# numericalEFT/MCIntegration.jl

Hardware: AMD Instinct MI355X
Metric: Msamples/sec (whole node), 16-D Gaussian :vegas (higher is better)
Workload: dtype f64

## Files before the change

### mcintegration.jl_amd/_lib.py

```python
import ctypes as C
import os

_PKG = os.path.dirname(os.path.abspath(__file__))
_SO = os.path.join(_PKG, "lib", "libmci_hip.so")

MCI_OK = 0
ERR_NAMES = {1: "INVALID", 2: "HIP", 3: "COMPILE", 4: "NORMALIZATION", 5: "HISTOGRAM", 6: "COMM", 7: "NO_DEVICE"}
CONTINUOUS, DISCRETE, FERMIK = 0, 1, 2
VEGAS, VEGASMC, MCMC = 0, 1, 2
ABI_VERSION = 5
SOLVERS = {"vegas": VEGAS, "vegasmc": VEGASMC, "mcmc": MCMC, VEGAS: VEGAS, VEGASMC: VEGASMC, MCMC: MCMC}

c_double_p = C.POINTER(C.c_double)
c_int32_p = C.POINTER(C.c_int32)


class MCIError(RuntimeError):
    def __init__(self, code, msg):
        super().__init__("[MCI_ERR_%s] %s" % (ERR_NAMES.get(code, code), msg))
        self.code = code


class LeafDesc(C.Structure):
    _fields_ = [("kind", C.c_int32), ("pool", C.c_int32), ("lower", C.c_double), ("upper", C.c_double),
# ... 113 lines not shown
    ("mci_mcmc_burnin", C.c_int64, [C.c_int64, C.c_int64, C.c_int32, C.c_int32, C.c_int32, C.c_double]),
    ("mci_mcmc_auto_chains", C.c_int64, [C.c_int64, C.c_int64, C.c_int32, C.c_int32, C.c_int32, C.c_int64, C.c_int64, C.c_int32]),
    ("mci_get_hold_histogram", C.c_int, [_VP, C.POINTER(C.c_uint64)]),
    ("mci_mcmc_launch_valid", C.c_int, [_VP, c_int32_p, c_int32_p, C.POINTER(C.c_int64), C.POINTER(C.c_int64)]),
    ("mci_iteration_discard", C.c_int, [_VP]),
    ("mci_get_block_means", C.c_int, [_VP, C.c_int32, c_double_p, C.POINTER(C.c_int64), c_int32_p]),
    ("mci_reset_block_log", C.c_int, [_VP]),
    ("mci_lineage_sums", None, [c_double_p, C.c_int64, C.c_int64, C.c_int64, c_double_p, C.c_int64, C.c_int64, c_double_p, c_double_p]),
    ("mci_maxdof", None, [c_int32_p, C.c_int32, C.c_int32, c_int32_p]),
    ("mci_mean_std", None, [c_double_p, c_double_p, C.c_int64, C.c_int64, c_double_p, c_double_p]),
    ("mci_average", None, [c_double_p, c_double_p, C.c_int64, C.c_int64, C.c_int64, c_double_p, c_double_p, c_double_p]),
    ("mci_do_reweight", None, [c_double_p, c_double_p, C.c_int64, C.c_double, c_double_p]),
    ("mci_version", C.c_char_p, []),
    ("mci_abi_version", C.c_int32, []),
]
DEBUG_SIGNATURES = [
    ("mci_debug_persist_words", C.c_int, [_VP, C.POINTER(C.c_uint64), C.c_int32]),
    ("mci_debug_walk_counts", C.c_int, [_VP, C.POINTER(C.c_int64)]),
    ("mci_debug_plant_wrong_decision", C.c_int, [_VP, C.c_int32]),
    ("mci_debug_persist_spin_ticks", C.c_int, [_VP, C.c_uint64]),
    ("mci_debug_override", C.c_int, [C.c_char_p, C.c_int64, C.c_int32]),
    ("mci_debug_compiler_id", C.c_int, [C.c_char_p, C.c_char_p, C.c_int32]),
    ("mci_debug_split_chunks", C.c_int, [_VP, C.POINTER(C.c_int64), C.POINTER(C.c_int64)]),
    ("mci_debug_strat_d", C.c_int, [_VP, c_double_p, C.c_int64]),
    ("mci_debug_strat_start_d", C.c_int, [_VP, c_double_p, C.c_int64]),
    ("mci_debug_strat_dump", C.c_int, [_VP, C.c_int64, c_double_p, c_double_p, C.POINTER(C.c_int64), c_double_p, c_double_p]),
    ("mci_debug_mcmc_policy", C.c_int, [C.c_int64, C.c_int64, C.c_int64, C.c_int64]),
    ("mci_debug_vegas_check", C.c_int, [_VP, C.c_int32, C.c_uint64, C.c_int64, C.c_int64, C.c_int64, C.c_int64, c_double_p, c_double_p, c_double_p, c_double_p,
                                        C.POINTER(C.c_int64)]),
    ("mci_debug_vegas_check_launches", C.c_int, [_VP, C.POINTER(C.c_int64)]),
    ("mci_debug_vegas_check_layout", C.c_int, [_VP, c_int32_p, c_int32_p, c_double_p, C.POINTER(C.c_uint64), c_int32_p]),
    ("mci_debug_sweep_workgroups", C.c_int, [_VP, C.c_int32]),
    ("mci_debug_sweep_threads", C.c_int, [_VP, C.c_int32]),
    ("mci_debug_sweep_last_launch", C.c_int, [_VP, c_int32_p, c_int32_p]),
    ("mci_debug_sweep_lds_bytes", C.c_int, [_VP, C.POINTER(C.c_int64)]),
]

_lib = None


def library_path():
    return _SO


def use_rocm_compiler(rocm=None):
    root = rocm or os.environ.get("ROCM_PATH") or "/opt/rocm"
# ... 55 lines not shown
```

### mcintegration.jl_amd/csrc/mci_debug.h

```cpp
#ifndef MCI_DEBUG_H
#define MCI_DEBUG_H
#include "../../include/mci.h"
#ifdef __cplusplus
extern "C" {
#endif
int mci_debug_persist_words(mci_problem *prob, unsigned long long *out, int32_t n);
int mci_debug_walk_counts(mci_problem *prob, int64_t *out);
int mci_debug_plant_wrong_decision(mci_problem *prob, int32_t on);
int mci_debug_persist_spin_ticks(mci_problem *prob, unsigned long long ticks);
int mci_debug_override(const char *key, int64_t value, int32_t on);
int mci_debug_split_chunks(const mci_problem *prob, int64_t *chunks, int64_t *bytes);
int mci_debug_strat_dump(mci_problem *prob, int64_t n, double *x, double *y, int64_t *h, double *jac, double *w);
int mci_debug_strat_d(mci_problem *prob, double *d, int64_t n);
int mci_debug_strat_start_d(mci_problem *prob, double *d, int64_t n);
int mci_debug_compiler_id(const char *set, char *out, int32_t n);
int mci_debug_mcmc_policy(int64_t pilot_steps, int64_t grow, int64_t carry_holds, int64_t carry_half_floors);
int mci_debug_vegas_check(mci_problem *prob, int32_t iteration, uint64_t seed, int64_t nevalperblock, int64_t block_lo, int64_t nblocks,
                          int64_t measurefreq, const double *x, const double *jac, const double *w, double *packed, int64_t *bad);
int mci_debug_vegas_check_launches(const mci_problem *prob, int64_t *launches);
int mci_debug_vegas_check_layout(const mci_problem *prob, int32_t *head, int32_t *draws, double *scales, uint64_t *own, int32_t *obs);
int mci_debug_sweep_workgroups(mci_problem *prob, int32_t g);
int mci_debug_sweep_threads(mci_problem *prob, int32_t threads);
int mci_debug_sweep_last_launch(const mci_problem *prob, int32_t *workgroups, int32_t *threads);
int mci_debug_sweep_lds_bytes(const mci_problem *prob, int64_t *bytes);
#ifdef __cplusplus
}
#endif
#endif
```

### mcintegration.jl_amd/csrc/mci_device.h

```cpp
#pragma once

namespace mci {

typedef unsigned int u32;
typedef unsigned long long u64;
typedef long long i64;

template <int I> struct IC { static constexpr int value = I; };

template <int B, int E, class F> __device__ __forceinline__ void static_for(F &&f) {
    if constexpr (B < E) {
        f(IC<B>{});
        static_for<B + 1, E>(f);
    }
}

struct u32x4 { u32 x, y, z, w; };

#ifndef MCI_PHILOX_ROUNDS
#define MCI_PHILOX_ROUNDS 10
#endif

template <bool IN_VGPR> struct RoundKeys {
    u32 a[MCI_PHILOX_ROUNDS], b[MCI_PHILOX_ROUNDS];
// ... 147 lines not shown
    int *store_curr;
    i64 store_cap;
    const double *carry_P;
    double *carry_w;
    i64 carry_total;
    double *store_P;
    struct HostStep {
        i64 ne, steps, nc;
        double *cx, *cprob, *cw, *cprobability;
        int *cbin;
        double *hx, *pprob, *pprop, *puacc;
        int *pbin, *pvi;
        double *cwabs;
        int *ccurr, *cit, *ctr;
        int *pnew, *put;
        int *hidx;
        int *done;
    } hs;
    const SpecNode *spec_tab;
    int spec_lanes, spec_maxacc;
    int spec_ntree, spec_first;
    float spec_accept[8];
    u64 *clock_out;
};

struct DumpArgs {
    const double *edges, *dacc, *ddist, *ud;
    double *x, *jac, *w;
    int soa;
    u64 seed;
    u32 iteration;
    i64 first_index;
    i64 n;
};

template <int CTRL, int ROW_MASK> __device__ __forceinline__ double dpp_read(double v) {
    const u64 u = (u64)__double_as_longlong(v);
    const int lo = __builtin_amdgcn_update_dpp(0, (int)(u32)u, CTRL, ROW_MASK, 0xf, false);
    const int hi = __builtin_amdgcn_update_dpp(0, (int)(u32)(u >> 32), CTRL, ROW_MASK, 0xf, false);
    return __longlong_as_double((long long)(((u64)(u32)hi << 32) | (u64)(u32)lo));
}
__device__ __forceinline__ double wave_scan_incl(double v) {
    v += dpp_read<0x111, 0xf>(v);
    v += dpp_read<0x112, 0xf>(v);
    v += dpp_read<0x114, 0xf>(v);
    v += dpp_read<0x118, 0xf>(v);
    v += dpp_read<0x142, 0xa>(v);
// ... 690 lines not shown
                });
            }
            __syncthreads();
        }
        static_for<0, Cfg::NTILE>([&](auto Tt) {
            constexpr int tt = decltype(Tt)::value;
            if (tile == tt) {
                double *hrow = a.part_hist + rowid * Cfg::NBIN + Cfg::tile_boff(tt);
                for (int i = tid; i < Cfg::tile_nbin(tt); i += T) {
                    constexpr int SB = (Cfg::DET != 0 || SUMMED) ? 1 : Cfg::HCOPY, SC = Cfg::DET != 0 ? Cfg::HTILE : 1;
                    double v = sH[i * SB];
                    if constexpr (!SUMMED)
                    static_for<1, Cfg::HCOPY>([&](auto Cc) { v += sH[i * SB + decltype(Cc)::value * SC]; });
                    if (!accum && a.hist_atomic) {
                        if (v != 0.0) global_add(&a.ghist[(rowid % a.hist_atomic) * Cfg::NBIN + Cfg::tile_boff(tt) + i], v);
                    } else
                    hrow[i] = accum ? hrow[i] + v : v;
                }
            }
        });
    }
}

struct WorkItem {
    i64 rowid, lb;
    int slice, tile;
};
template <class Cfg> __device__ __forceinline__ WorkItem work_item(const BatchArgs &a) {
    WorkItem w;
#ifdef MCI_WORK_ITEM_FROM_CALLER
    w.tile = 0;
    w.rowid = a.chunk_lo;
#else
    w.tile = Cfg::NTILE == 1 ? 0 : (int)(blockIdx.x % Cfg::NTILE);
    w.rowid = Cfg::NTILE == 1 ? (i64)blockIdx.x : (i64)(blockIdx.x / Cfg::NTILE);
#endif
    w.lb = w.rowid / a.wg_per_block;
    w.slice = (int)(w.rowid % a.wg_per_block);
    return w;
}

template <class Cfg, bool SPLIT = false> __device__ __forceinline__ void vegas_batch(const BatchArgs &a) {
    extern __shared__ __attribute__((aligned(16))) double smem[];
    const int tid = threadIdx.x, T = blockDim.x;
    constexpr bool NOHIST = SPLIT && Cfg::SPLIT_ALL != 0;
    constexpr bool EC = Cfg::EC_DOUBLES > 0 && (NOHIST || !SPLIT);
// ... 20 lines not shown
        static_for<0, Cfg::NLEAF>([&](auto Lf) {
            constexpr int l = decltype(Lf)::value;
            if constexpr (Cfg::leaf_kind(l) == 0 && Cfg::leaf_ecoff(l) >= 0)
                for (int i = tid; i <= Cfg::leaf_nbin(l); i += T) sEC[Cfg::leaf_ecoff(l) + i] = a.edges[Cfg::leaf_eoff(l) + i];
        });
        t.EC = sEC;
    }
    __syncthreads();
    if constexpr (Mode<Cfg>::EDGE_LDS) t.E = sE;
    else t.E = a.edges;
    t.DA = sDA;
    t.DD = sDD;

    WorkItem wi = work_item<Cfg>(a);
    if constexpr (SPLIT) {
        wi.tile = 0;
        wi.rowid = (i64)blockIdx.x;
        wi.lb = wi.rowid / a.wg_per_block;
        wi.slice = (int)(wi.rowid % a.wg_per_block);
    }
    const int slice = wi.slice, tile = wi.tile;
    const i64 B = a.block_lo + wi.lb;
    const u32 stream = a.iteration * 8u + STREAM_VEGAS;
    const i64 stride = (i64)a.wg_per_block * T;

    double acc[Cfg::NW];
    static_for<0, Cfg::NW>([&](auto I) { acc[decltype(I)::value] = 0.0; });
    double extra[Cfg::NCOLS - Cfg::NOBS];
    static_for<0, Cfg::NCOLS - Cfg::NOBS>([&](auto I) { extra[decltype(I)::value] = 0.0; });

#ifndef MCI_PIPE_VGPR_KEYS
#define MCI_PIPE_VGPR_KEYS 0
#endif
    constexpr bool KV = MCI_PIPE_VGPR_KEYS != 0 && pipe_eligible<Cfg>() && !SPLIT && Cfg::EC_DOUBLES == 0;
    constexpr int DPC = Cfg::RNG_BITS == 32 ? 4 : 2;
    const RoundKeys<KV> keys = make_round_keys<KV>((u32)a.seed, (u32)(a.seed >> 32));
    const i64 mfreq = a.measurefreq;
    const i64 n_lo = SPLIT ? a.chunk_lo : 0, n_hi = SPLIT ? a.chunk_hi : a.neval_per_block;
    i64 mrem = mfreq == 1 ? 0 : (n_lo + (i64)slice * T + tid + 1) % mfreq;
    const i64 mstep = mfreq == 1 ? 0 : stride % mfreq;
    constexpr bool PHASED = Cfg::L1_PHASE > 0 && Cfg::HOST_INTEGRAND == 0 && gather_draw_count<Cfg, EC>() > 0;
    auto run = [&](auto TT, auto MF1c) {
    constexpr bool MF1 = decltype(MF1c)::value != 0;
    auto process = [&](const i64 n, const Sample<Cfg> &s, double *defer_wh = nullptr) {
        double w[Cfg::NW];
        if constexpr (Cfg::HOST_INTEGRAND != 0) {
            const i64 hidx = wi.lb * a.neval_per_block + n;
            static_for<0, Cfg::NW>([&](auto Q) { w[decltype(Q)::value] = a.host_w[decltype(Q)::value * a.tile_stride + hidx]; });
        } else {
            Cfg::integrand(s.x, w, a.ud, -1);
        }
        extra[Cols<Cfg>::NEVAL - Cfg::NOBS] += 1.0;
        bool domeasure = true;
        if constexpr (!MF1) {
            domeasure = mrem == 0;
            mrem += mstep;
            mrem = mrem >= mfreq ? mrem - mfreq : mrem;
        }
        if constexpr (Cfg::HOST_MEASURE != 0) {
            const i64 hidx = wi.lb * a.neval_per_block + n;
            static_for<0, Cfg::NDRAW>([&](auto K) { a.host_mx[decltype(K)::value * a.tile_stride + hidx] = s.x[decltype(K)::value]; });
            static_for<0, Cfg::NW>([&](auto Q) {
                constexpr int q = decltype(Q)::value;
                a.host_relw[q * a.tile_stride + hidx] = domeasure ? w[q] * s.jaci[q / Cfg::NCOMP] : 0.0;
            });
            if (domeasure) extra[Cols<Cfg>::NORM - Cfg::NOBS] += 1.0;
        } else if (domeasure) {
            double relw[Cfg::NW];
            static_for<0, Cfg::NW>([&](auto Q) { constexpr int q = decltype(Q)::value; relw[q] = w[q] * s.jaci[q / Cfg::NCOMP]; });
            measure<Cfg>(s.x, s.bin, relw, a.ud, acc, obs_wave<Cfg>(sO));
            extra[Cols<Cfg>::NORM - Cfg::NOBS] += 1.0;
        }
        double wh[Cfg::NI];
        static_for<0, Cfg::NI>([&](auto I) {
            constexpr int i = decltype(I)::value;
            const double wj = absw<Cfg, i>(w) * s.jac;
            wh[i] = wj * wj;
        });
        if (defer_wh) {
            static_for<0, Cfg::NI>([&](auto I) { defer_wh[decltype(I)::value] = wh[decltype(I)::value]; });
        } else if constexpr (!NOHIST) hist_update<Cfg, decltype(TT)::value>(s, wh, sH, a.ghist, tile);
        if constexpr (SPLIT) {
            const i64 idx = wi.lb * a.chunk_len + (n - n_lo);
            static_for<0, Cfg::NI>([&](auto I) { a.tile_w[decltype(I)::value * a.tile_stride + idx] = wh[decltype(I)::value]; });
            constexpr int NWORD = tdraw_words<Cfg>();
            static_for<0, NWORD>([&](auto J) { a.tile_bins[decltype(J)::value * a.tile_stride + idx] = s.word[decltype(J)::value]; });
        }
    };
    if constexpr (PHASED) {
        const i64 n0 = n_lo + (i64)slice * T + tid, first = n_lo + (i64)slice * T;
        const i64 jfull = first + T <= n_hi ? (n_hi - first - T) / stride + 1 : 0;
        i64 n = n0;
        for (i64 j = 0; j < jfull; ++j, n += stride) {
            Sample<Cfg> sm;
// ... 2 lines not shown
            __builtin_amdgcn_sched_barrier(0);
            draw_rest_phase<Cfg, EC, KV, DPC>(t, keys, stream, index, sm);
            process(n, sm);
            __builtin_amdgcn_sched_barrier(0);
        }
        for (; n < n_hi; n += stride) {
            Sample<Cfg> s;
            draw_sample<Cfg, EC, KV, DPC>(t, keys, stream, (u64)(B * a.neval_per_block + n), s);
            process(n, s);
        }
    } else if constexpr (pipe_eligible<Cfg>() && !SPLIT && !EC) {
        const u64 first = (u64)(B * a.neval_per_block);
        const bool uniform_hi = (first >> 32) == ((first + (u64)a.neval_per_block - 1ull) >> 32);
        auto loop = [&](auto UNIc) {
            constexpr bool UNI = decltype(UNIc)::value != 0;
            PendingHist<Cfg> pa, pb;
            static_for<0, Cfg::NDRAW>([&](auto K) { pa.bin[decltype(K)::value] = 0; });
            static_for<0, Cfg::NI>([&](auto I) { pa.wh[decltype(I)::value] = 0.0; });
            auto flush = [&](const PendingHist<Cfg> &q) {
                static_for<0, Cfg::NDRAW>([&](auto K) { hist_add_draw<Cfg, decltype(K)::value>(q.bin[decltype(K)::value], q.wh, sH); });
            };
            PhiloxHead<pipe_blocks<Cfg, DPC>()> head;
            if constexpr (UNI) head = make_philox_head<pipe_blocks<Cfg, DPC>()>((u32)a.seed, (u32)(a.seed >> 32), (u32)(first >> 32), stream);
            i64 n = (i64)slice * T + tid;
            for (; n + stride < a.neval_per_block; n += 2 * stride) {
                {
                    Sample<Cfg> s;
                    draw_sample_pipe<Cfg, KV, DPC, UNI>(keys, head, stream, first + (u64)n, s, pa, pb, sH);
                    process(n, s, pb.wh);
                }
                {
                    Sample<Cfg> s;
                    draw_sample_pipe<Cfg, KV, DPC, UNI>(keys, head, stream, first + (u64)(n + stride), s, pb, pa, sH);
                    process(n + stride, s, pa.wh);
                }
            }
            if (n < a.neval_per_block) {
                Sample<Cfg> s;
                draw_sample_pipe<Cfg, KV, DPC, UNI>(keys, head, stream, first + (u64)n, s, pa, pb, sH);
                process(n, s, pb.wh);
                flush(pb);
            } else flush(pa);
        };
        if (uniform_hi) loop(IC<1>{});
        else loop(IC<0>{});
    } else {
        for (i64 n = n_lo + (i64)slice * T + tid; n < n_hi; n += stride) {
            Sample<Cfg> s;
            draw_sample<Cfg, EC, KV, DPC>(t, keys, stream, (u64)(B * a.neval_per_block + n), s);
            process(n, s);
        }
    }
    };
#ifndef MCI_MF_ONLY
#define MCI_MF_ONLY 0
#endif
    auto run_mf = [&](auto TT) { run(TT, IC<(MCI_MF_ONLY != 0 ? 1 : 0)>{}); };
    const bool stamp = !SPLIT && Cfg::NTILE == 1 && a.clock_out != nullptr && blockIdx.x == 0 && tid < 64;
    u64 ck0 = 0ull, rt0 = 0ull;
    if (stamp) {
        ck0 = __builtin_amdgcn_s_memtime();
        rt0 = __builtin_amdgcn_s_memrealtime();
    }
    if constexpr (Cfg::NTILE == 1 || SPLIT) run_mf(IC<0>{});
    else static_for<0, Cfg::NTILE>([&](auto TT) { if (tile == decltype(TT)::value) run_mf(TT); });
// ... 1484 lines not shown
```

### mcintegration.jl_amd/csrc/mci_host_iteration.h

```cpp
int mci_iteration_run(mci_problem *p, int32_t solver, int64_t nevalperblock, int64_t block_lo, int64_t block_hi,
                      int32_t iteration, uint64_t seed, int64_t measurefreq, int64_t nchain, double thermal_ratio) {
    if (p->ctx->offline) return fail(MCI_ERR_NO_DEVICE, "offline context: no device to run on");
    if (solver != MCI_VEGAS && solver != MCI_VEGASMC && solver != MCI_MCMC) return fail(MCI_ERR_INVALID, "Solver %d is not supported!", solver);
    const bool auto_chains = nchain <= 0;
    if (measurefreq <= 0) return fail(MCI_ERR_INVALID, "measurefreq must be positive");
    const int64_t nblocks = block_hi - block_lo;
    if (nblocks < 1 || nevalperblock < 1) return fail(MCI_ERR_INVALID, "empty iteration");
    if (p->has_fermik && solver != MCI_MCMC) return fail(MCI_ERR_INVALID, "FermiK variables work with solver=:mcmc only");
    if (p->strat.on) {
        if (solver != MCI_VEGAS) return fail(MCI_ERR_INVALID, "stratification works with solver = :vegas only (mci_set_stratification_off first)");
        return strat_run(p, nevalperblock, block_lo, block_hi, iteration, seed, measurefreq);
    }
    const int kern = (p->in_self_check && p->check_slot >= 0 && solver == MCI_VEGAS) ? p->check_slot : kslot(solver, measurefreq);
    int rc = (solver == MCI_VEGAS || p->deterministic || p->shape.host_integrand || p->spec_lanes == 1) ? compile_solver(p, kern) : MCI_OK;
    if (rc) return rc;
    if (solver == MCI_VEGAS && !p->in_self_check && !p->vegas_check_done[kern == kSlotVegasAny ? 1 : 0] &&
        (rc = vegas_check_gate(p, kern, nevalperblock, block_lo, block_hi, iteration, seed, measurefreq)))
        return rc;
    if (solver == MCI_VEGAS && (rc = compile_solver(p, kern))) return rc;
    if (solver == MCI_VEGAS && p->shape.host_integrand && (rc = ensure_dump(p))) return rc;
    if ((rc = flush_merge(p))) return rc;
    HIPCHK(hipSetDevice(p->ctx->device));
    const auto &s = p->shape;
    int T = solver_threads(p, solver);
// ... 75 lines not shown
        spec_maxacc = p->spec_tab_maxacc;
        units = nchain * G;
        T_launch = units >= 256 ? 256 : (int)((units + 63) / 64) * 64;
    }
    if (G == 1 && (rc = compile_solver(p, kern))) return rc;
    p->launch.last_spec_lanes = G;
    p->launch.last_spec_maxacc = spec_maxacc;
    int wpb = p->wg_per_block;
    if (G > 1) {
        if (wpb <= 0) wpb = (int)((2048 + nblocks - 1) / nblocks);
        const int64_t maxw = (units + T_launch - 1) / T_launch;
        if (wpb > maxw) wpb = (int)maxw;
        if (wpb < 1) wpb = 1;
    } else
    if (wpb <= 0) {
        const int64_t big = T >= 1024 ? 1024 : T >= 512 ? 2048 : 4096;
        int64_t target = (units * nblocks >= (int64_t)1 << 25 && p->lds_bytes <= 32 * 1024) ? big : 2048;
        if (solver == MCI_VEGAS && units * nblocks < ((int64_t)1 << 22) && target > 256) target = 256;
        if (solver == MCI_VEGAS && units * nblocks * s.ndraw < ((int64_t)1 << 19) && target > 64) target = 64;
        wpb = (int)((target + nblocks - 1) / nblocks);
        const int64_t maxw = (units + T - 1) / T;
        if (wpb > maxw) wpb = (int)maxw;
        if (wpb < 1) wpb = 1;
    }
    const bool hist_lds = (s.table_mode == 0 || s.table_mode == 3);
    const bool split = solver == MCI_VEGAS && s.ntile > 1;
    if (!split && wpb * s.ntile > 4096 / nblocks && s.ntile > 1) wpb = (int)(4096 / nblocks / s.ntile) > 0 ? (int)(4096 / nblocks / s.ntile) : 1;
    const int64_t nrows = nblocks * wpb;
    const bool atomic_flush = solver == MCI_VEGAS && hist_lds && s.ntile == 1 && atomic_rows_ok(p) && nrows <= kAtomicRows && !s.host_integrand;
    const int64_t nwg = split ? nrows : nrows * s.ntile;
    if ((rc = ensure_capacity(p, nrows, nblocks))) return rc;
    if (solver != MCI_VEGAS && nrows > p->cap_pa) {
        if (p->d_part_pa) (void)hipFree(p->d_part_pa);
        p->d_part_pa = nullptr;
        p->cap_pa = 0;
        HIPCHK(hipMalloc((void **)&p->d_part_pa, (size_t)nrows * 2 * p->npa * sizeof(double)));
        p->cap_pa = nrows;
    }
    int64_t chunk_len = nevalperblock, nchunks = 1;
    if (split) {
        const int64_t words = p->tdraw_words > 0 ? p->tdraw_words : 1;
        const int64_t bytes = (int64_t)s.ni * 8 + words * 4;
        if (!s.host_integrand && !s.host_measure) {
            int64_t cap = (int64_t)1 << 27;
            if (cap * bytes > (int64_t)7500000000) cap = (int64_t)7500000000 / bytes;
            if (g_over.split_chunk.on && g_over.split_chunk.v > 0) cap = g_over.split_chunk.v;
// ... 265 lines not shown
            HIPCHK(hipHostMalloc((void **)&p->h_mx, (size_t)n * s.ndraw * sizeof(double), hipHostMallocDefault));
            HIPCHK(hipHostMalloc((void **)&p->h_mrelw, (size_t)n * nw * sizeof(double), hipHostMallocDefault));
            HIPCHK(hipHostMalloc((void **)&p->h_midx, (size_t)n * sizeof(int32_t), hipHostMallocDefault));
            p->cap_hmeas = n;
        }
        if (nblocks * s.nobs > p->cap_mobs) {
            if (p->d_mobs) (void)hipFree(p->d_mobs);
            p->d_mobs = nullptr;
            HIPCHK(hipMalloc((void **)&p->d_mobs, (size_t)nblocks * s.nobs * sizeof(double)));
            p->cap_mobs = nblocks * s.nobs;
        }
        a.host_mx = p->d_mx;
        a.host_relw = p->d_mrelw;
        a.host_midx = p->d_midx;
        a.hm_first = hm_first;
        a.hm_count = hm_count;
        a.hm_stride = nblocks * hm_n;
        if (solver != MCI_VEGAS) {
            HIPCHK(hipMemsetAsync(p->d_mx, 0, (size_t)n * s.ndraw * sizeof(double), p->ctx->stream));
            HIPCHK(hipMemsetAsync(p->d_mrelw, 0, (size_t)n * hm_rows * sizeof(double), p->ctx->stream));
            HIPCHK(hipMemsetAsync(p->d_midx, 0xFF, (size_t)n * sizeof(int32_t), p->ctx->stream));
        }
    }
    void *args[] = {&a};
    hipFunction_t f = p->f_solver[G > 1 ? (solver == MCI_VEGASMC ? kSlotVegasmcSpec : kSlotMcmcSpec) : kern];
    hipStream_t st = p->ctx->stream;
    const int slot = (int)(p->launch.launches % mci_problem::kEvRing);
    p->launch.time_this_launch = p->kernel_timing > 0 || (p->kernel_timing < 0 && nblocks * nevalperblock >= ((int64_t)1 << 20));
    if (p->launch.time_this_launch && solver == MCI_VEGAS) {
        if (!p->d_clocks) {
            HIPCHK(hipMalloc((void **)&p->d_clocks, (size_t)2 * mci_problem::kEvRing * sizeof(unsigned long long)));
            HIPCHK(hipMemsetAsync(p->d_clocks, 0, (size_t)2 * mci_problem::kEvRing * sizeof(unsigned long long), st));
        }
        a.clock_out = p->d_clocks + 2 * slot;
    }
    if (p->launch.time_this_launch) HIPCHK(hipEventRecord(p->evs[2 * slot], st));
    if (solver != MCI_VEGAS && s.host_integrand) {
        const int64_t nc = nblocks * nchain, steps = nevalperblock / nchain;
        const int nw = s.ni * s.ncomp, nd = s.ndraw;
        if (nc >= ((int64_t)1 << 31) || steps + nburn >= ((int64_t)1 << 31) - 1) return fail(MCI_ERR_INVALID, "too many chains or steps for the host-closure path");
        if (nc > p->cap_hstep) {
            if (p->d_hstep) (void)hipFree(p->d_hstep);
            p->d_hstep = nullptr;
            p->cap_hstep = 0;
            HIPCHK(hipMalloc(&p->d_hstep, (size_t)nc * ((3 * nd + nw + 4) * sizeof(double) + (2 * nd + 7) * sizeof(int)) + 16));
            p->cap_hstep = nc;
// ... 367 lines not shown
```

### mcintegration.jl_amd/csrc/mci_host_jit.h

```cpp
enum { kSlotVegasAny = 3, kSlotDump = 4, kSlotVegasmcSpec = 5, kSlotMcmcSpec = 6 };
static int kslot(int solver, int64_t measurefreq) { return solver == MCI_VEGAS && measurefreq != 1 ? kSlotVegasAny : solver; }
static int slot_solver(int slot) { return slot == kSlotVegasAny ? MCI_VEGAS : slot == kSlotVegasmcSpec ? MCI_VEGASMC : slot == kSlotMcmcSpec ? MCI_MCMC : slot; }

namespace {
struct Candidate {
    std::string src;
    int threads = 256;
    std::vector<char> code;
    std::string log, path;
    bool cached = false;
    int rc = 0;
    long vgprs() const { return mcijit::kernel_vgprs(code, "mci_vegas_batch"); }
    long scratch() const { return mcijit::kernel_scratch_bytes(code, "mci_vegas_batch"); }
};
void compile_all(std::vector<Candidate *> &cs) {
    std::vector<std::thread> th;
    for (size_t i = 1; i < cs.size(); ++i)
        th.emplace_back([c = cs[i]] { c->rc = mcijit::compile(c->src, c->threads, c->code, c->log, c->cached, &c->path); });
    if (!cs.empty()) cs[0]->rc = mcijit::compile(cs[0]->src, cs[0]->threads, cs[0]->code, cs[0]->log, cs[0]->cached, &cs[0]->path);
    for (auto &t : th) t.join();
}
}

static int load_slot(mci_problem *p, int slot, Candidate &c, int64_t lds) {
// ... 499 lines not shown
}

int mci_debug_plant_wrong_decision(mci_problem *p, int32_t on) {
    if (!p) return fail(MCI_ERR_INVALID, "NULL argument");
    p->debug_wrong_decision = on != 0;
    return MCI_OK;
}

int mci_debug_override(const char *key, int64_t value, int32_t on) {
    Override *o = override_slot(key);
    if (!o) return fail(MCI_ERR_INVALID, "no such override: %s", key ? key : "(null)");
    o->on = on != 0;
    o->v = value;
    return MCI_OK;
}

int mci_debug_split_chunks(const mci_problem *p, int64_t *chunks, int64_t *bytes) {
    if (!p) return fail(MCI_ERR_INVALID, "NULL argument");
    if (chunks) *chunks = p->launch.last_split_chunks;
    if (bytes) *bytes = p->launch.last_split_bytes;
    return MCI_OK;
}

int mci_debug_compiler_id(const char *set, char *out, int32_t n) {
    if (set) mcijit::compiler_id_override() = set;
    if (out && n > 0) snprintf(out, (size_t)n, "%s", mcijit::compiler_id().c_str());
    return MCI_OK;
}

int mci_debug_mcmc_policy(int64_t pilot_steps, int64_t grow, int64_t carry_holds, int64_t carry_half_floors) {
    if (pilot_steps > 0) mci_problem::kMcmcPilotSteps = pilot_steps;
    if (grow > 0) mci_problem::kMcmcGrow = grow;
    if (carry_holds > 0) mci_problem::kMcmcCarryHolds = carry_holds;
    if (carry_half_floors > 0) mci_problem::kMcmcCarryHalfFloors = carry_half_floors;
    return MCI_OK;
}

int mci_debug_persist_spin_ticks(mci_problem *p, unsigned long long ticks) {
    if (!p || ticks == 0) return fail(MCI_ERR_INVALID, "bad argument");
    p->persist_spin_ticks = ticks;
    return MCI_OK;
}

int mci_set_deterministic(mci_problem *p, int32_t on) {
    if (!p) return fail(MCI_ERR_INVALID, "NULL argument");
    const bool want = on != 0;
// ... 118 lines not shown
```

### mcintegration.jl_amd/csrc/mci_host_problem.h

```cpp
int mci_problem_create(mci_ctx *ctx, const mci_problem_desc *d, mci_problem **out) {
    if (!ctx || !d || !out) return fail(MCI_ERR_INVALID, "NULL argument");
    if (d->nleaf < 1 || d->npool < 1 || d->nintegrand < 1) return fail(MCI_ERR_INVALID, "At least one integrand is required.");
    if (d->nintegrand > 31) return fail(MCI_ERR_INVALID, "at most 31 integrands are supported");
    mci_problem *p = new mci_problem();
    p->ctx = ctx;
    p->npool = d->npool;
    p->ni = d->nintegrand;
    const int Nd = p->ni + 1;
    p->dof.assign((size_t)Nd * p->npool, 0);
    for (int i = 0; i < p->ni * p->npool; ++i) {
        if (d->dof[i] < 0) { delete p; return fail(MCI_ERR_INVALID, "dof must be non-negative"); }
        p->dof[i] = d->dof[i];
    }
    p->maxdof.assign(p->npool, 0);
    mci_maxdof(p->dof.data(), Nd, p->npool, p->maxdof.data());
    p->pool_leaf0.assign(p->npool, -1);
    p->pool_nleaf.assign(p->npool, 0);
    auto &s = p->shape;
    int eoff = 0, aoff = 0, doff = 0, boff = 0;
    for (int l = 0; l < d->nleaf; ++l) {
        const mci_leaf_desc &ld = d->leaves[l];
        if (ld.pool < 0 || ld.pool >= p->npool) { delete p; return fail(MCI_ERR_INVALID, "leaf %d: pool out of range", l); }
        if (p->pool_leaf0[ld.pool] < 0) p->pool_leaf0[ld.pool] = l;
        else if (p->pool_leaf0[ld.pool] + p->pool_nleaf[ld.pool] != l) { delete p; return fail(MCI_ERR_INVALID, "leaves of pool %d are not contiguous", ld.pool); }
// ... 333 lines not shown
        if (p->strat.module) (void)hipModuleUnload(p->strat.module);
        if (p->sweep.module) (void)hipModuleUnload(p->sweep.module);
        if (p->sweep.leaves.module) (void)hipModuleUnload(p->sweep.leaves.module);
        strat_free_buffers(p);
        if (p->d_persist) (void)hipFree(p->d_persist);
    }
    persist_job_drop(p);
    if (!p->ctx->offline) {
        if (p->d_goal) (void)hipFree(p->d_goal);
        if (p->d_part_pa) (void)hipFree(p->d_part_pa);
        if (p->d_hold) (void)hipFree(p->d_hold);
        for (int b = 0; b < 2; ++b) {
            if (p->d_chain_x[b]) (void)hipFree(p->d_chain_x[b]);
            if (p->d_chain_curr[b]) (void)hipFree(p->d_chain_curr[b]);
        }
        if (p->d_reweight_used) (void)hipFree(p->d_reweight_used);
        if (p->d_carry_W) (void)hipFree(p->d_carry_W);
        if (p->d_carry_src) (void)hipFree(p->d_carry_src);
        if (p->d_spec_tab) (void)hipFree(p->d_spec_tab);
        for (int b = 0; b < 2; ++b)
            if (p->d_chain_P[b]) (void)hipFree(p->d_chain_P[b]);
        if (p->d_carry_w) (void)hipFree(p->d_carry_w);
        if (p->d_clocks) (void)hipFree(p->d_clocks);
        if (p->d_edges_backup) (void)hipFree(p->d_edges_backup);
        if (p->h_hold) (void)hipHostFree(p->h_hold);
        if (p->h_hold_d) (void)hipHostFree(p->h_hold_d);
        if (p->h_log) (void)hipHostFree(p->h_log);
        if (p->hold_ev) (void)hipEventDestroy(p->hold_ev);
        if (p->d_blocklog) (void)hipFree(p->d_blocklog);
        for (auto &e : p->cevs) (void)hipEventDestroy(e);
        if (p->d_hx) (void)hipFree(p->d_hx);
        if (p->d_hstep) (void)hipFree(p->d_hstep);
        if (p->h_hidx) (void)hipHostFree(p->h_hidx);
        if (p->d_hw) (void)hipFree(p->d_hw);
        if (p->h_hx) (void)hipHostFree(p->h_hx);
        if (p->h_hw) (void)hipHostFree(p->h_hw);
        tile_release(p);
        if (p->d_mx) (void)hipFree(p->d_mx);
        if (p->d_mrelw) (void)hipFree(p->d_mrelw);
        if (p->d_mobs) (void)hipFree(p->d_mobs);
        if (p->h_mx) (void)hipHostFree(p->h_mx);
        if (p->h_mrelw) (void)hipHostFree(p->h_mrelw);
        if (p->d_midx) (void)hipFree(p->d_midx);
        if (p->h_midx) (void)hipHostFree(p->h_midx);
        for (auto &e : p->evs) (void)hipEventDestroy(e);
    }
// ... 130 lines not shown
    return hc;
}

static int64_t vegas_lds(const mci_problem *p) {
    const auto &s = p->shape;
    return (s.ec_doubles > 0 ? p->lds_bytes_k1 : p->lds_bytes) + (int64_t)s.htile * 8 * (s.hcopy - 1);
}

static const int64_t kAtomicRows = 256;
static bool atomic_rows_ok(const mci_problem *p) { return !p->deterministic && kAtomicRows > 0; }

static int solver_threads(const mci_problem *p, int solver) {
    if (p->deterministic && p->threads_det[solver]) return p->threads_det[solver];
    return solver == MCI_VEGAS && p->threads_vegas ? p->threads_vegas : p->threads;
}
static int64_t det_lds(const mci_problem *p, int threads) {
    const auto &s = p->shape;
    return p->lds_bytes + ((int64_t)s.htile + s.nobs) * 8 * (threads / 64 - 1);
}
static int64_t solver_lds(const mci_problem *p, int solver) {
    if (p->deterministic) return det_lds(p, solver_threads(p, solver));
    return solver == MCI_VEGAS ? vegas_lds(p) : p->lds_bytes;
}
```

### mcintegration.jl_amd/csrc/mci_host_types.h

```cpp
namespace {

struct Id128 { char b[128]; };
struct Rccl {
    void *h = nullptr;
    int (*GetUniqueId)(void *) = nullptr;
    int (*CommInitRank)(void **, int, Id128 , int) = nullptr;
    int (*AllReduce)(const void *, void *, size_t, int, int, void *, hipStream_t) = nullptr;
    int (*CommDestroy)(void *) = nullptr;
    const char *(*GetErrorString)(int) = nullptr;
};
Rccl g_rccl;
const int kNcclFloat64 = 8, kNcclSum = 0;

int find_loaded_rccl(struct dl_phdr_info *info, size_t, void *out) {
    const char *n = info->dlpi_name;
    if (n && strstr(n, "librccl.so")) {
        *(std::string *)out = n;
        return 1;
    }
    return 0;
}

int rccl_load() {
    if (g_rccl.h) return MCI_OK;
// ... 151 lines not shown
    double *d_reweight_used = nullptr, *d_carry_W = nullptr;
    int *d_carry_src = nullptr;
    int64_t cap_carry_src = 0, cap_carry_W = 0;
    unsigned long long *d_clocks = nullptr;
    std::vector<hipEvent_t> evs;
    static const int kEvRing = 512;
    int log_row = 0;
    double *h_log = nullptr;
    size_t cap_hlog = 0;
    hipModule_t module_persist = nullptr;
    hipFunction_t f_persist = nullptr;
    bool persist_compiled = false, persist_failed = false;
    std::string persist_code_object;
    int persist_threads = 256;
    struct PersistJob;
    PersistJob *persist_job = nullptr;
    unsigned long long *d_persist = nullptr;
    double *d_edges_backup = nullptr;
    unsigned long long persist_arrive = 0, persist_done = 0;
    unsigned long long persist_spin_ticks = 200000000ull;
    int persistent = -1;
    bool last_persistent = false;
    static const int kGroups = mci::kMergeGroups;
    static const int64_t kChainFill = 131072;
    static int64_t kMcmcPilotSteps, kMcmcGrow;
    static int64_t kMcmcCarryHolds, kMcmcCarryHalfFloors;
    struct LaunchState {
        int last_wg = 0, last_threads = 0, last_nblocks = 0;
        int64_t last_samples = 0;
        int64_t last_nchain = 0;
        int last_spec_lanes = 1, last_spec_maxacc = 0;
        bool last_carried = false;
        int64_t last_split_chunks = 0, last_split_bytes = 0;
        int64_t launches = 0;
        bool time_this_launch = true;
        bool ev_valid[kEvRing] = {};
        bool clock_valid[kEvRing] = {};
        int chain_cur = 0;
        bool chain_valid = false;
        int chain_solver = -1, chain_iteration = -1;
        int64_t chain_lo = 0, chain_hi = 0, chain_nchain = 0;
        int64_t chain_ntrain = 0;
        int64_t blk_rows = 0, blk_stride = 0, blk_lo = -1;
        int blk_carried = 0;
        int64_t hold_max = 0;
        int64_t hold_len = 0;
        int64_t hold_prev = 0;
        bool hold_valid = false;
        bool hold_measured = false;
        bool mcmc_warm = false;
        bool hold_inflight = false;
        bool hold_from_packed = false;
        bool hold_deferred = false;
        bool hold_ext_pending = false;
        int64_t hold_launches = 0;
// ... 46 lines not shown
        int grid = 0;
        int want_threads = 0;
        int last_grid = 0, last_threads = 0;
        int leaves_mode = 0;
        struct Unit {
            bool compiled = false;
            int threads = 0;
            hipModule_t module = nullptr;
            hipFunction_t f = nullptr;
            std::string code_object;
        } leaves;
    } sweep;
};

static const int kRepeatStride = 16384, kMaxRepeats = 7;

int64_t mci_problem::kMcmcPilotSteps = 4096;
int64_t mci_problem::kMcmcGrow = 2;
int64_t mci_problem::kMcmcCarryHolds = 4;
int64_t mci_problem::kMcmcCarryHalfFloors = 2;

namespace {
struct Override { bool on = false; int64_t v = 0; };
struct Overrides { Override table_mode, hist_tile_bins, no_split_all, l1_phase, train_walk, hist_copies, fresh_floors, fresh_burnin_pct, spec_self_check, split_chunk, vegas_self_check; } g_over;
Override *override_slot(const char *key) {
    if (!key) return nullptr;
    if (!strcmp(key, "table_mode")) return &g_over.table_mode;
    if (!strcmp(key, "hist_tile_bins")) return &g_over.hist_tile_bins;
    if (!strcmp(key, "no_split_all")) return &g_over.no_split_all;
    if (!strcmp(key, "l1_phase")) return &g_over.l1_phase;
    if (!strcmp(key, "train_walk")) return &g_over.train_walk;
    if (!strcmp(key, "hist_copies")) return &g_over.hist_copies;
    if (!strcmp(key, "fresh_floors")) return &g_over.fresh_floors;
    if (!strcmp(key, "fresh_burnin_pct")) return &g_over.fresh_burnin_pct;
    if (!strcmp(key, "spec_self_check")) return &g_over.spec_self_check;
    if (!strcmp(key, "split_chunk")) return &g_over.split_chunk;
    if (!strcmp(key, "vegas_self_check")) return &g_over.vegas_self_check;
    return nullptr;
}
}

static void persist_job_drop(mci_problem *p);
namespace { void persist_orphans_join(); }
static const size_t kPersistWords = 8 + 3 * 8 * 8 + 16;

namespace {

int tile_alloc(mci_problem *p, size_t bytes) {
    mci_ctx *c = p->ctx;
    void *base = nullptr;
    {
        std::lock_guard<std::mutex> g(c->spare_mu);
        if (c->spare && c->spare_bytes >= bytes && c->spare_bytes <= 2 * bytes + ((size_t)64 << 20)) {
            base = c->spare;
            p->tile_bytes = c->spare_bytes;
            c->spare = nullptr;
            c->spare_bytes = 0;
        }
    }
    if (!base) {
// ... 124 lines not shown
}

int hold_consume(mci_problem *p) {
    if (!p->launch.hold_inflight) return MCI_OK;
    HIPCHK(hipEventSynchronize(p->hold_ev));
    p->launch.hold_inflight = false;
    int top = -1;
    for (int b = 0; b < 64; ++b)
        if (p->launch.hold_from_packed ? p->h_hold_d[b] > 0.5 : p->h_hold[b] != 0ull) top = b;
    if (top >= 0) {
        p->launch.hold_prev = p->launch.mcmc_warm ? p->launch.hold_max : 0;
        p->launch.hold_max = (int64_t)1 << top;
        p->launch.hold_len = p->launch.hold_len_inflight;
        p->launch.hold_valid = p->launch.hold_len >= (p->launch.hold_carried_inflight ? mci_problem::kMcmcCarryHolds : 16) * p->launch.hold_max;
        if (p->launch.hold_valid) p->launch.mcmc_warm = true;
    }
    return MCI_OK;
}

void drop_modules(mci_problem *p) {
    p->vegas_planned = p->vegas_keys = p->vegas_wide = false;
    p->vegas_check_done[0] = p->vegas_check_done[1] = false;
    p->f_dump = nullptr;
    for (int k = 0; k < mci_problem::kSlots; ++k) {
        p->compiled[k] = false;
        if (p->module[k]) {
            (void)hipModuleUnload(p->module[k]);
            p->module[k] = nullptr;
        }
    }
    p->persist_compiled = p->persist_failed = false;
    persist_job_drop(p);
    p->f_persist = nullptr;
    if (p->module_persist) {
        (void)hipModuleUnload(p->module_persist);
        p->module_persist = nullptr;
    }
    p->strat.compiled = false;
    p->strat.f = nullptr;
    if (p->strat.module) {
        (void)hipModuleUnload(p->strat.module);
        p->strat.module = nullptr;
    }
    p->sweep.compiled = false;
    p->sweep.f = nullptr;
    if (p->sweep.module) {
// ... 34 lines not shown
```

### mcintegration.jl_amd/engine.py

```python
import atexit
import ctypes as C
import weakref

import numpy as np

from . import _lib
from ._lib import LeafDesc, ProblemDesc, c_double_p, c_int32_p, check, lib
from .integrand import HostIntegrand, HostMeasure, Integrand, Measure
from .variables import ContinuousVar, FermiK

_ctx_cache = {}


def _dp(a):
    return a.ctypes.data_as(c_double_p)


def context(device=0):
    if device not in _ctx_cache:
        p = C.c_void_p()
        check(lib().mci_ctx_create(device, C.byref(p)))
        _ctx_cache[device] = p
    return _ctx_cache[device]

# ... 535 lines not shown
        nd, ni = int(head[0]), int(head[1])
        draws, scales = (C.c_int32 * (6 * max(nd, 1)))(), (C.c_double * max(nd, 1))()
        own, obs = (C.c_uint64 * max(ni, 1))(), (C.c_int32 * (3 * max(ni, 1)))()
        check(lib().mci_debug_vegas_check_layout(self.p, head, draws, scales, own, obs))
        keys = ("kind", "off", "doff", "nbin", "boff", "hist")
        return dict(ndraw=nd, ni=ni, ncomp=int(head[2]), nobs=int(head[3]), ncols=int(head[4]), nbin=int(head[5]), covered=bool(head[6]),
                    with_obs=bool(head[7]),
                    draws=[dict(zip(keys, [int(draws[6 * k + j]) for j in range(6)]), scale=float(scales[k])) for k in range(nd)],
                    integrands=[dict(own=int(own[i]), obs_off=int(obs[3 * i]), obs_nbin=int(obs[3 * i + 1]), obs_bin_draw=int(obs[3 * i + 2]))
                                for i in range(ni)])

    def compile_chain_speculation(self, solver):
        check(lib().mci_compile_chain_speculation(self.p, _lib.SOLVERS[solver]))

    def set_train_walk(self, mode):
        check(lib().mci_debug_plant_wrong_decision(self.p, 1 if mode in ("serial_wrong_decision", 3) else 0))
        check(lib().mci_set_train_walk(self.p, {"auto": -1, "scan": 0, "serial": 1, "serial_general": 2, "serial_wrong_decision": 1, -1: -1, 0: 0, 1: 1, 2: 2, 3: 1}[mode]))

    def walk_counts(self):
        out = (C.c_int64 * 2)()
        check(lib().mci_debug_walk_counts(self.p, out))
        return int(out[0]), int(out[1])

    def split_chunks(self):
        n, b = C.c_int64(), C.c_int64()
        check(lib().mci_debug_split_chunks(self.p, C.byref(n), C.byref(b)))
        return int(n.value), int(b.value)

    def integrate(self, solver, neval, niter=10, block=16, ignore=-1, adapt=True, gamma=1.0, measurefreq=1, seed=1234,
                  nchain=0, first_iteration=0, thermal_ratio=0.1, reweight_goal=None):
        goal = None
        if reweight_goal is not None:
            self._goal = np.ascontiguousarray(reweight_goal, dtype=np.float64)
            goal = _dp(self._goal)
        a = _lib.IntegrateArgs(_lib.SOLVERS[solver], int(neval), int(niter), int(block), int(ignore), 1 if adapt else 0,
                               float(gamma), int(measurefreq), int(seed), int(nchain), int(first_iteration),
                               float(thermal_ratio), goal)
        n = self.nobs
        im, ie = np.zeros((niter, n)), np.zeros((niter, n))
        m, s, c2 = np.zeros(n), np.zeros(n), np.zeros(n)
        vis = np.zeros(self.config.N + 1)
        r = _lib.ResultC(niter, n, _dp(im), _dp(ie), _dp(m), _dp(s), _dp(c2), 0, 0.0, _dp(vis), 0, 0)
        check(lib().mci_integrate(self.p, C.byref(a), C.byref(r)))
        dn, dl = C.c_int64(), C.c_int32()
        check(lib().mci_last_integrate_discarded(self.p, C.byref(dn), C.byref(dl)))
        out = dict(mean=m, stdev=s, chi2=c2, iter_mean=im, iter_std=ie, neval=r.neval, seconds=r.seconds, visited=vis,
# ... 268 lines not shown
```

Before: 75720.

## Add atomic-cursor dynamic work distribution for VEGAS pipe kernel

Replaces the static strided split of samples across workgroups in the VEGAS sampling loop with a per-block global atomic ticket counter. Wavefronts pull chunks of 128-sample units, large chunks first and shrinking geometrically toward single units at the end (guided self-scheduling), and the workgroup count is sized to device residency. It targets tail imbalance and idle CUs when waves finish unevenly. In exchange it adds atomic traffic and per-chunk bookkeeping, and the eval/norm counts are now accumulated once per thread rather than per sample. It is enabled only for large continuous-variable problems that meet the residency and size thresholds.

```diff
diff --git a/mcintegration.jl_amd/_lib.py b/mcintegration.jl_amd/_lib.py
--- a/mcintegration.jl_amd/_lib.py
+++ b/mcintegration.jl_amd/_lib.py
@@ -159,6 +159,7 @@
     ("mci_debug_override", C.c_int, [C.c_char_p, C.c_int64, C.c_int32]),
     ("mci_debug_compiler_id", C.c_int, [C.c_char_p, C.c_char_p, C.c_int32]),
     ("mci_debug_split_chunks", C.c_int, [_VP, C.POINTER(C.c_int64), C.POINTER(C.c_int64)]),
+    ("mci_debug_vegas_cursor", C.c_int, [_VP, C.POINTER(C.c_int32), C.POINTER(C.c_uint64)]),
     ("mci_debug_strat_d", C.c_int, [_VP, c_double_p, C.c_int64]),
     ("mci_debug_strat_start_d", C.c_int, [_VP, c_double_p, C.c_int64]),
     ("mci_debug_strat_dump", C.c_int, [_VP, C.c_int64, c_double_p, c_double_p, C.POINTER(C.c_int64), c_double_p, c_double_p]),
diff --git a/mcintegration.jl_amd/csrc/mci_debug.h b/mcintegration.jl_amd/csrc/mci_debug.h
--- a/mcintegration.jl_amd/csrc/mci_debug.h
+++ b/mcintegration.jl_amd/csrc/mci_debug.h
@@ -13,6 +13,7 @@
 int mci_debug_strat_dump(mci_problem *prob, int64_t n, double *x, double *y, int64_t *h, double *jac, double *w);
 int mci_debug_strat_d(mci_problem *prob, double *d, int64_t n);
 int mci_debug_strat_start_d(mci_problem *prob, double *d, int64_t n);
+int mci_debug_vegas_cursor(const mci_problem *prob, int32_t *used, uint64_t *base);
 int mci_debug_compiler_id(const char *set, char *out, int32_t n);
 int mci_debug_mcmc_policy(int64_t pilot_steps, int64_t grow, int64_t carry_holds, int64_t carry_half_floors);
 int mci_debug_vegas_check(mci_problem *prob, int32_t iteration, uint64_t seed, int64_t nevalperblock, int64_t block_lo, int64_t nblocks,
diff --git a/mcintegration.jl_amd/csrc/mci_device.h b/mcintegration.jl_amd/csrc/mci_device.h
--- a/mcintegration.jl_amd/csrc/mci_device.h
+++ b/mcintegration.jl_amd/csrc/mci_device.h
@@ -193,7 +193,11 @@
     int spec_ntree, spec_first;
     float spec_accept[8];
     u64 *clock_out;
+    u64 *cursor;
+    u64 cursor_base;
+    u32 cursor_log2_big, cursor_ones;
 };
+constexpr int kCursorStride = 32;
 
 struct DumpArgs {
     const double *edges, *dacc, *ddist, *ud;
@@ -930,6 +934,37 @@
     }
 }
 
+struct CursorRule {
+    u64 units;
+    u32 waves;
+    u32 log2_big, ones;
+};
+__host__ __device__ inline u64 cursor_ones(const CursorRule &r) { return (u64)r.ones * r.waves; }
+__host__ __device__ inline u64 cursor_tickets(const CursorRule &r) {
+    if (r.units <= cursor_ones(r)) return r.units;
+    u64 rem = r.units - cursor_ones(r), n = cursor_ones(r);
+    for (u32 l = 1; l < r.log2_big; ++l) {
+        const u64 level = (u64)r.waves << l;
+        if (rem <= level) return n + ((rem + (1ull << l) - 1ull) >> l);
+        n += r.waves;
+        rem -= level;
+    }
+    return n + ((rem + (1ull << r.log2_big) - 1ull) >> r.log2_big);
+}
+__host__ __device__ inline void cursor_range(const CursorRule &r, u64 ntickets, u64 t, u64 &u0, u64 &u1) {
+    u64 q = ntickets - 1ull - t, e, z = 1ull;
+    if (q < cursor_ones(r)) e = q;
+    else {
+        q -= cursor_ones(r);
+        u32 l = 1;
+        for (; l < r.log2_big && q >= r.waves; ++l) q -= r.waves;
+        z = 1ull << l;
+        e = (u64)r.waves * (r.ones + z - 2ull) + q * z;
+    }
+    u1 = r.units - e;
+    u0 = e + z < r.units ? r.units - e - z : 0ull;
+}
+
 struct WorkItem {
     i64 rowid, lb;
     int slice, tile;
@@ -996,7 +1031,8 @@
     const int slice = wi.slice, tile = wi.tile;
     const i64 B = a.block_lo + wi.lb;
     const u32 stream = a.iteration * 8u + STREAM_VEGAS;
-    const i64 stride = (i64)a.wg_per_block * T;
+    const bool pulled = pipe_eligible<Cfg>() && !SPLIT && !EC && a.cursor != nullptr;
+    const i64 stride = pulled ? 64 : (i64)a.wg_per_block * T;
 
     double acc[Cfg::NW];
     static_for<0, Cfg::NW>([&](auto I) { acc[decltype(I)::value] = 0.0; });
@@ -1016,7 +1052,8 @@
     constexpr bool PHASED = Cfg::L1_PHASE > 0 && Cfg::HOST_INTEGRAND == 0 && gather_draw_count<Cfg, EC>() > 0;
     auto run = [&](auto TT, auto MF1c) {
     constexpr bool MF1 = decltype(MF1c)::value != 0;
-    auto process = [&](const i64 n, const Sample<Cfg> &s, double *defer_wh = nullptr) {
+    auto process = [&](const i64 n, const Sample<Cfg> &s, double *defer_wh = nullptr, auto... counted) {
+        constexpr bool COUNTED = sizeof...(counted) > 0;
         double w[Cfg::NW];
         if constexpr (Cfg::HOST_INTEGRAND != 0) {
             const i64 hidx = wi.lb * a.neval_per_block + n;
@@ -1024,7 +1061,7 @@
         } else {
             Cfg::integrand(s.x, w, a.ud, -1);
         }
-        extra[Cols<Cfg>::NEVAL - Cfg::NOBS] += 1.0;
+        if constexpr (!COUNTED) extra[Cols<Cfg>::NEVAL - Cfg::NOBS] += 1.0;
         bool domeasure = true;
         if constexpr (!MF1) {
             domeasure = mrem == 0;
@@ -1043,7 +1080,7 @@
             double relw[Cfg::NW];
             static_for<0, Cfg::NW>([&](auto Q) { constexpr int q = decltype(Q)::value; relw[q] = w[q] * s.jaci[q / Cfg::NCOMP]; });
             measure<Cfg>(s.x, s.bin, relw, a.ud, acc, obs_wave<Cfg>(sO));
-            extra[Cols<Cfg>::NORM - Cfg::NOBS] += 1.0;
+            if constexpr (!(COUNTED && MF1)) extra[Cols<Cfg>::NORM - Cfg::NOBS] += 1.0;
         }
         double wh[Cfg::NI];
         static_for<0, Cfg::NI>([&](auto I) {
@@ -1092,25 +1129,70 @@
             };
             PhiloxHead<pipe_blocks<Cfg, DPC>()> head;
             if constexpr (UNI) head = make_philox_head<pipe_blocks<Cfg, DPC>()>((u32)a.seed, (u32)(a.seed >> 32), (u32)(first >> 32), stream);
-            i64 n = (i64)slice * T + tid;
-            for (; n + stride < a.neval_per_block; n += 2 * stride) {
-                {
-                    Sample<Cfg> s;
-                    draw_sample_pipe<Cfg, KV, DPC, UNI>(keys, head, stream, first + (u64)n, s, pa, pb, sH);
-                    process(n, s, pb.wh);
+            CursorRule rule;
+            rule.units = (u64)((a.neval_per_block + 127) >> 7);
+            rule.waves = (u32)a.wg_per_block * (u32)(T >> 6);
+            rule.log2_big = a.cursor_log2_big;
+            rule.ones = a.cursor_ones;
+            const u64 ntickets = pulled ? cursor_tickets(rule) : 0ull;
+            u64 *const word = a.cursor + wi.lb * kCursorStride;
+            auto pull = [&]() -> u64 {
+                u64 r = 0ull;
+                if ((tid & 63) == 0) {
+                    u64 addr = (u64)word;
+                    asm volatile("" : "+v"(addr));
+                    typedef __attribute__((address_space(1))) u64 global_u64;
+                    r = __hip_atomic_fetch_add((global_u64 *)addr, 1ull, __ATOMIC_RELAXED, __HIP_MEMORY_SCOPE_AGENT);
                 }
-                {
-                    Sample<Cfg> s;
-                    draw_sample_pipe<Cfg, KV, DPC, UNI>(keys, head, stream, first + (u64)(n + stride), s, pb, pa, sH);
-                    process(n + stride, s, pa.wh);
+                return r;
+            };
+            auto ticket = [&](u64 r) -> u64 {
+                const u32 lo = (u32)__builtin_amdgcn_readfirstlane((int)(u32)r), hi = (u32)__builtin_amdgcn_readfirstlane((int)(u32)(r >> 32));
+                return (((u64)hi << 32) | lo) - a.cursor_base;
+            };
+            i64 n = (i64)slice * T + tid, lim = a.neval_per_block;
+            u32 trips = 0u;
+            u64 next = 0ull;
+            if (pulled) {
+                next = pull();
+                n = lim = 0;
+            }
+            for (;;) {
+                if (pulled) {
+                    const u64 t = ticket(next);
+                    if (t >= ntickets) break;
+                    next = pull();
+                    u64 u0, u1;
+                    cursor_range(rule, ntickets, t, u0, u1);
+                    n = (i64)(u0 << 7) + (tid & 63);
+                    lim = (i64)(u1 << 7) < a.neval_per_block ? (i64)(u1 << 7) : a.neval_per_block;
+                    if constexpr (!MF1) mrem = (n + 1) % mfreq;
                 }
-            }
-            if (n < a.neval_per_block) {
+                for (; n + stride < lim; n += 2 * stride) {
+                    {
+                        Sample<Cfg> s;
+                        draw_sample_pipe<Cfg, KV, DPC, UNI>(keys, head, stream, first + (u64)n, s, pa, pb, sH);
+                        process(n, s, pb.wh, 0);
+                    }
+                    {
+                        Sample<Cfg> s;
+                        draw_sample_pipe<Cfg, KV, DPC, UNI>(keys, head, stream, first + (u64)(n + stride), s, pb, pa, sH);
+                        process(n + stride, s, pa.wh, 0);
+                    }
+                    trips += 1u;
+                }
+                if (!pulled) break;
+            }
+            double count = 2.0 * (double)trips;
+            if (n < lim) {
                 Sample<Cfg> s;
                 draw_sample_pipe<Cfg, KV, DPC, UNI>(keys, head, stream, first + (u64)n, s, pa, pb, sH);
-                process(n, s, pb.wh);
+                process(n, s, pb.wh, 0);
                 flush(pb);
+                count += 1.0;
             } else flush(pa);
+            extra[Cols<Cfg>::NEVAL - Cfg::NOBS] += count;
+            if constexpr (MF1) extra[Cols<Cfg>::NORM - Cfg::NOBS] += count;
         };
         if (uniform_hi) loop(IC<1>{});
         else loop(IC<0>{});
diff --git a/mcintegration.jl_amd/csrc/mci_host_iteration.h b/mcintegration.jl_amd/csrc/mci_host_iteration.h
--- a/mcintegration.jl_amd/csrc/mci_host_iteration.h
+++ b/mcintegration.jl_amd/csrc/mci_host_iteration.h
@@ -121,6 +121,21 @@
         const int64_t maxw = (units + T - 1) / T;
         if (wpb > maxw) wpb = (int)maxw;
         if (wpb < 1) wpb = 1;
+    }
+    bool cursor = false;
+    if (solver == MCI_VEGAS && G == 1 && !p->in_self_check && vegas_pipe_unit(p) && !(g_over.vegas_cursor.on && g_over.vegas_cursor.v == 0)) {
+        const bool forced = g_over.vegas_cursor.on && g_over.vegas_cursor.v == 1;
+        if (forced) cursor = true;
+        else if (p->wg_per_block <= 0 && units * nblocks >= ((int64_t)1 << 25)) {
+            int resident = 0;
+            if ((rc = cursor_resident(p, kern, T, &resident))) return rc;
+            if (resident >= nblocks && (resident / nblocks) * nblocks > kAtomicRows) {
+                cursor = true;
+                wpb = (int)(resident / nblocks);
+                const int64_t maxw = (units + T - 1) / T;
+                if (wpb > maxw) wpb = (int)maxw;
+            }
+        }
     }
     const bool hist_lds = (s.table_mode == 0 || s.table_mode == 3);
     const bool split = solver == MCI_VEGAS && s.ntile > 1;
@@ -432,6 +447,31 @@
             HIPCHK(hipMemsetAsync(p->d_midx, 0xFF, (size_t)n * sizeof(int32_t), p->ctx->stream));
         }
     }
+    if (cursor) {
+        mci::CursorRule r;
+        r.units = (mci::u64)((nevalperblock + 127) >> 7);
+        r.waves = (mci::u32)(wpb * (T / 64));
+        r.log2_big = (mci::u32)(g_over.cursor_log2_big.on && g_over.cursor_log2_big.v >= 1 && g_over.cursor_log2_big.v <= 16 ? g_over.cursor_log2_big.v : mci_problem::kCursorLog2Big);
+        r.ones = (mci::u32)(g_over.cursor_ones.on && g_over.cursor_ones.v >= 1 && g_over.cursor_ones.v <= 4096 ? g_over.cursor_ones.v : mci_problem::kCursorOnes);
+        if (nblocks != p->cursor_nblocks) {
+            if (nblocks > p->cap_cursor) {
+                if (p->d_cursor) (void)hipFree(p->d_cursor);
+                p->d_cursor = nullptr;
+                p->cap_cursor = 0;
+                HIPCHK(hipMalloc((void **)&p->d_cursor, (size_t)nblocks * mci::kCursorStride * sizeof(unsigned long long)));
+                p->cap_cursor = nblocks;
+            }
+            HIPCHK(hipMemsetAsync(p->d_cursor, 0, (size_t)nblocks * mci::kCursorStride * sizeof(unsigned long long), p->ctx->stream));
+            p->cursor_nblocks = nblocks;
+            p->cursor_base = 0;
+        }
+        a.cursor = p->d_cursor;
+        a.cursor_base = p->cursor_base;
+        a.cursor_log2_big = r.log2_big;
+        a.cursor_ones = r.ones;
+        p->cursor_base += mci::cursor_tickets(r) + r.waves;
+    }
+    p->launch.last_cursor = cursor;
     void *args[] = {&a};
     hipFunction_t f = p->f_solver[G > 1 ? (solver == MCI_VEGASMC ? kSlotVegasmcSpec : kSlotMcmcSpec) : kern];
     hipStream_t st = p->ctx->stream;
diff --git a/mcintegration.jl_amd/csrc/mci_host_jit.h b/mcintegration.jl_amd/csrc/mci_host_jit.h
--- a/mcintegration.jl_amd/csrc/mci_host_jit.h
+++ b/mcintegration.jl_amd/csrc/mci_host_jit.h
@@ -545,6 +545,13 @@
     return MCI_OK;
 }
 
+int mci_debug_vegas_cursor(const mci_problem *p, int32_t *used, uint64_t *base) {
+    if (!p) return fail(MCI_ERR_INVALID, "NULL argument");
+    if (used) *used = p->launch.last_cursor ? 1 : 0;
+    if (base) *base = p->cursor_base;
+    return MCI_OK;
+}
+
 int mci_debug_compiler_id(const char *set, char *out, int32_t n) {
     if (set) mcijit::compiler_id_override() = set;
     if (out && n > 0) snprintf(out, (size_t)n, "%s", mcijit::compiler_id().c_str());
diff --git a/mcintegration.jl_amd/csrc/mci_host_problem.h b/mcintegration.jl_amd/csrc/mci_host_problem.h
--- a/mcintegration.jl_amd/csrc/mci_host_problem.h
+++ b/mcintegration.jl_amd/csrc/mci_host_problem.h
@@ -379,6 +379,7 @@
             if (p->d_chain_P[b]) (void)hipFree(p->d_chain_P[b]);
         if (p->d_carry_w) (void)hipFree(p->d_carry_w);
         if (p->d_clocks) (void)hipFree(p->d_clocks);
+        if (p->d_cursor) (void)hipFree(p->d_cursor);
         if (p->d_edges_backup) (void)hipFree(p->d_edges_backup);
         if (p->h_hold) (void)hipHostFree(p->h_hold);
         if (p->h_hold_d) (void)hipHostFree(p->h_hold_d);
@@ -555,3 +556,28 @@
     if (p->deterministic) return det_lds(p, solver_threads(p, solver));
     return solver == MCI_VEGAS ? vegas_lds(p) : p->lds_bytes;
 }
+
+static bool vegas_pipe_unit(const mci_problem *p) {
+    const auto &s = p->shape;
+    if (p->vegas_conservative || p->deterministic || s.det) return false;
+    if (s.ndraw < 8 || s.ndraw > 16 || !s.pair_table || s.table_mode != 0 || s.ntile != 1) return false;
+    if (s.host_integrand || s.host_measure || s.ec_doubles > 0) return false;
+    for (const auto &l : p->leaves)
+        if (l.kind != 0) return false;
+    return true;
+}
+static int cursor_resident(mci_problem *p, int kern, int threads, int *out) {
+    hipFunction_t f = p->f_solver[kern];
+    const int64_t lds = solver_lds(p, MCI_VEGAS);
+    if (f != p->cursor_occ_f || threads != p->cursor_occ_threads || lds != p->cursor_occ_lds) {
+        int per_cu = 0, cus = 0;
+        HIPCHK(hipModuleOccupancyMaxActiveBlocksPerMultiprocessor(&per_cu, f, threads, (size_t)lds));
+        HIPCHK(hipDeviceGetAttribute(&cus, hipDeviceAttributeMultiprocessorCount, p->ctx->device));
+        p->cursor_occ_f = f;
+        p->cursor_occ_threads = threads;
+        p->cursor_occ_lds = lds;
+        p->cursor_occ_resident = per_cu * cus;
+    }
+    *out = p->cursor_occ_resident;
+    return MCI_OK;
+}
diff --git a/mcintegration.jl_amd/csrc/mci_host_types.h b/mcintegration.jl_amd/csrc/mci_host_types.h
--- a/mcintegration.jl_amd/csrc/mci_host_types.h
+++ b/mcintegration.jl_amd/csrc/mci_host_types.h
@@ -197,6 +197,13 @@
     int persistent = -1;
     bool last_persistent = false;
     static const int kGroups = mci::kMergeGroups;
+    static const int kCursorLog2Big = 4, kCursorOnes = 4;
+    unsigned long long *d_cursor = nullptr;
+    int64_t cap_cursor = 0, cursor_nblocks = 0;
+    unsigned long long cursor_base = 0;
+    hipFunction_t cursor_occ_f = nullptr;
+    int cursor_occ_threads = 0, cursor_occ_resident = 0;
+    int64_t cursor_occ_lds = 0;
     static const int64_t kChainFill = 131072;
     static int64_t kMcmcPilotSteps, kMcmcGrow;
     static int64_t kMcmcCarryHolds, kMcmcCarryHalfFloors;
@@ -206,6 +213,7 @@
         int64_t last_nchain = 0;
         int last_spec_lanes = 1, last_spec_maxacc = 0;
         bool last_carried = false;
+        bool last_cursor = false;
         int64_t last_split_chunks = 0, last_split_bytes = 0;
         int64_t launches = 0;
         bool time_this_launch = true;
@@ -298,7 +306,7 @@
 
 namespace {
 struct Override { bool on = false; int64_t v = 0; };
-struct Overrides { Override table_mode, hist_tile_bins, no_split_all, l1_phase, train_walk, hist_copies, fresh_floors, fresh_burnin_pct, spec_self_check, split_chunk, vegas_self_check; } g_over;
+struct Overrides { Override table_mode, hist_tile_bins, no_split_all, l1_phase, train_walk, hist_copies, fresh_floors, fresh_burnin_pct, spec_self_check, split_chunk, vegas_self_check, vegas_cursor, cursor_log2_big, cursor_ones; } g_over;
 Override *override_slot(const char *key) {
     if (!key) return nullptr;
     if (!strcmp(key, "table_mode")) return &g_over.table_mode;
@@ -312,6 +320,9 @@
     if (!strcmp(key, "spec_self_check")) return &g_over.spec_self_check;
     if (!strcmp(key, "split_chunk")) return &g_over.split_chunk;
     if (!strcmp(key, "vegas_self_check")) return &g_over.vegas_self_check;
+    if (!strcmp(key, "vegas_cursor")) return &g_over.vegas_cursor;
+    if (!strcmp(key, "cursor_log2_big")) return &g_over.cursor_log2_big;
+    if (!strcmp(key, "cursor_ones")) return &g_over.cursor_ones;
     return nullptr;
 }
 }
@@ -482,6 +493,7 @@
     p->vegas_planned = p->vegas_keys = p->vegas_wide = false;
     p->vegas_check_done[0] = p->vegas_check_done[1] = false;
     p->f_dump = nullptr;
+    p->cursor_occ_f = nullptr;
     for (int k = 0; k < mci_problem::kSlots; ++k) {
         p->compiled[k] = false;
         if (p->module[k]) {
diff --git a/mcintegration.jl_amd/engine.py b/mcintegration.jl_amd/engine.py
--- a/mcintegration.jl_amd/engine.py
+++ b/mcintegration.jl_amd/engine.py
@@ -581,6 +581,11 @@
         check(lib().mci_debug_walk_counts(self.p, out))
         return int(out[0]), int(out[1])
 
+    def last_launch_cursor(self):
+        used, base = C.c_int32(0), C.c_uint64(0)
+        check(lib().mci_debug_vegas_cursor(self.p, C.byref(used), C.byref(base)))
+        return bool(used.value), int(base.value)
+
     def split_chunks(self):
         n, b = C.c_int64(), C.c_int64()
         check(lib().mci_debug_split_chunks(self.p, C.byref(n), C.byref(b)))
```

Result: faster. 76700 (median of 6 runs) (+1.3%).
